# preethamam/AutomaticPanoramicImageStitching-AutoPanoStitch-MATLAB

Measured on AMD Instinct MI355X. Metric: MPix/s end-to-end stitch (SIFT->blend), 64x4K images, higher is better.
Workload: dtype f32; 1 GPU

## Files before the change

automaticpanoramicimagestitching-autopanostitch-matlab_amd/csrc/aps_internal.h:

```cpp
#pragma once
#include <hip/hip_runtime.h>
#include <type_traits>

#include <cstdarg>
#include <cstdint>
#include <cstdio>
#include <cstring>
#include <stdexcept>
#include <string>
#include <vector>

#include "../../include/aps.h"

namespace aps {

struct Error : std::exception {
    int code;
    std::string msg;
    Error(int c, std::string m) : code(c), msg(std::move(m)) {}
    const char* what() const noexcept override { return msg.c_str(); }
};

[[noreturn]] void fail(int code, const char* fmt, ...) __attribute__((format(printf, 2, 3)));
void set_last_error(const char* s);

#define APS_HIP(expr)                                                                       \
    do {                                                                                    \
        hipError_t e_ = (expr);                                                             \
        if (e_ != hipSuccess)                                                               \
            ::aps::fail(e_ == hipErrorOutOfMemory ? APS_E_OOM : APS_E_DEVICE,               \
                        "%s failed: %s (%s:%d)", #expr, hipGetErrorString(e_), __FILE__,    \
                        __LINE__);                                                          \
    } while (0)

#define APS_REQUIRE(cond, code, ...)                   \
    do {                                               \
        if (!(cond)) ::aps::fail((code), __VA_ARGS__); \
    } while (0)

template <class F>
inline int guarded(F&& f) {
    try {
        f();
        return APS_OK;
    } catch (const Error& e) {
        set_last_error(e.msg.c_str());
        return e.code;
    } catch (const std::bad_alloc&) {
        set_last_error("host allocation failed");
        return APS_E_OOM;
    } catch (const std::exception& e) {
        set_last_error(e.what());
        return APS_E_INTERNAL;
    } catch (...) {
        set_last_error("unknown exception");
        return APS_E_INTERNAL;
    }
}

struct Ctx {
    int device = -1;
    hipStream_t own_stream = nullptr;
    hipStream_t user_stream = nullptr;
    bool use_user_stream = false;
    int own_priority = 0;
    hipEvent_t ev0 = nullptr, ev1 = nullptr;
    struct Block {
        void* p;
        size_t bytes;
        bool used;
    };
    std::vector<Block> blocks;
    hipStream_t stream() const { return use_user_stream ? user_stream : own_stream; }
};

Ctx& ctx();
inline hipStream_t stream() { return ctx().stream(); }

void* ws_alloc(size_t bytes);
void ws_free(void* p);
size_t ws_idle_bytes();

template <class T>
struct Ws {
    T* p = nullptr;
    size_t n = 0;
    Ws() = default;
    explicit Ws(size_t count) { alloc(count); }
    Ws(const Ws&) = delete;
    Ws& operator=(const Ws&) = delete;
    Ws(Ws&& o) noexcept : p(o.p), n(o.n) { o.p = nullptr; }
    Ws& operator=(Ws&& o) noexcept {
        if (this != &o) {
            reset();
            p = o.p;
            n = o.n;
            o.p = nullptr;
        }
        return *this;
    }
    ~Ws() { reset(); }
    void alloc(size_t count) {
        reset();
        n = count;
        p = static_cast<T*>(ws_alloc((count ? count : 1) * sizeof(T)));
    }
    void reset() {
        if (p) ws_free(p);
        p = nullptr;
    }
    T* get() const { return p; }
    operator T*() const { return p; }
};

bool is_device_ptr(const void* p);

template <class T>
struct In {
    const T* d = nullptr;
    Ws<T> tmp;
    In() = default;
    In(const T* p, size_t count) { bind(p, count); }
    void bind(const T* p, size_t count) {
        if (count == 0 || p == nullptr) {
            d = p;
            return;
        }
        if (is_device_ptr(p)) {
            d = p;
        } else {
            tmp.alloc(count);
            APS_HIP(hipMemcpyAsync(tmp.p, p, count * sizeof(T), hipMemcpyHostToDevice, stream()));
            d = tmp.p;
        }
    }
    const T* get() const { return d; }
    operator const T*() const { return d; }
};

template <class T>
struct Out {
    T* d = nullptr;
    T* host = nullptr;
    size_t n = 0;
    Ws<T> tmp;
    Out() = default;
    Out(T* p, size_t count) { bind(p, count); }
    void bind(T* p, size_t count) {
        n = count;
        if (p == nullptr) return;
        if (count == 0 || is_device_ptr(p)) {
            d = p;
        } else {
            host = p;
            tmp.alloc(count);
            d = tmp.p;
        }
    }
    void commit(size_t count = SIZE_MAX) {
        if (!host) return;
        if (count > n) count = n;
        if (count) {
            APS_HIP(hipMemcpyAsync(host, d, count * sizeof(T), hipMemcpyDeviceToHost, stream()));
            APS_HIP(hipStreamSynchronize(stream()));
        }
    }
    void commit_2d(size_t width, size_t rows, size_t ld) {
        if (!host || width == 0 || rows == 0) return;
        if (ld == width || rows == 1) return commit(width * rows);
        APS_HIP(hipMemcpy2DAsync(host, ld * sizeof(T), d, ld * sizeof(T), width * sizeof(T), rows, hipMemcpyDeviceToHost, stream()));
        APS_HIP(hipStreamSynchronize(stream()));
    }
    T* get() const { return d; }
    operator T*() const { return d; }
    bool present() const { return d != nullptr; }
};

struct Prof {
    int slot = -1;
    void* ev_b = nullptr;
    explicit Prof(const char* name);
    ~Prof();
};

inline void check_launch(const char* what) {
    hipError_t e = hipGetLastError();
    if (e != hipSuccess) fail(APS_E_DEVICE, "launch of %s failed: %s", what, hipGetErrorString(e));
}

inline size_t matrix_extent(int64_t n, int64_t ld, int64_t cols, int layout) {
    return layout == APS_ROWMAJOR ? (size_t)(n - 1) * ld + cols : (size_t)(cols - 1) * ld + n;
}

template <class Off, class Key>
__device__ __forceinline__ int last_at_or_below_by(Off&& off, int n, Key key) {
    int lo = 0, hi = n - 1;
    while (lo < hi) {
        const int mid = (lo + hi + 1) >> 1;
        if (off(mid) <= key) lo = mid; else hi = mid - 1;
    }
    return lo;
}
template <class T, class Key>
__device__ __forceinline__ int last_at_or_below(const T* __restrict__ off, int n, Key key) {
    return last_at_or_below_by([off](int j) { return off[j]; }, n, key);
}

struct SlotTable {
    std::vector<int64_t> job_off;
    int64_t slots = 0;
};
SlotTable slot_table(const std::vector<int64_t>& off, int a, int b, bool every_j);
void screened_block_top3(const float* X_dev, int64_t ld, int layout, const std::vector<int64_t>& block_off, const SlotTable& table,
                         uint32_t* t3_idx, float* t3_d, float* t3_b);
struct GlobalSets {
    struct Impl;
    Impl* impl = nullptr;
    GlobalSets() = default;
    GlobalSets(const GlobalSets&) = delete;
    GlobalSets& operator=(const GlobalSets&) = delete;
    ~GlobalSets();
};
int64_t screened_global_top3(const float* X_dev, int64_t ld, int layout, const std::vector<int64_t>& img_off, int img_a, int img_b,
                             float ratio, const SlotTable& table, const int64_t* d_img_off, const int64_t* d_job_off, GlobalSets& sets,
                             uint32_t* t3_idx, float* t3_d, float* t3_b, uint8_t* dismissed);

struct PopcOp {
    __host__ __device__ unsigned int operator()(unsigned long long v) const {
#if defined(__HIP_DEVICE_COMPILE__)
        return (unsigned int)__popcll(v);
#else
        return (unsigned int)__builtin_popcountll(v);
#endif
    }
};

inline unsigned cdiv(size_t a, size_t b) { return static_cast<unsigned>((a + b - 1) / b); }

template <int I, int N, class F>
__device__ __forceinline__ void static_for(F&& f) {
    if constexpr (I < N) {
        f(std::integral_constant<int, I>{});
        static_for<I + 1, N>(f);
    }
}


}
```

automaticpanoramicimagestitching-autopanostitch-matlab_amd/csrc/core.hip:

```cpp
#include <atomic>
#include <cstdlib>
#include <mutex>

#include <cstring>

#include "aps_internal.h"

namespace aps {

static thread_local std::string g_err;
static thread_local Ctx g_ctx;
static std::atomic<int> g_default_device{-1};

void set_last_error(const char* s) { g_err = s ? s : ""; }

void fail(int code, const char* fmt, ...) {
    char buf[1024];
    va_list ap;
    va_start(ap, fmt);
    vsnprintf(buf, sizeof buf, fmt, ap);
    va_end(ap);
    throw Error(code, buf);
}

static bool device_is_gfx950(int dev) {
    hipDeviceProp_t prop;
    if (hipGetDeviceProperties(&prop, dev) != hipSuccess) return false;
    return std::strncmp(prop.gcnArchName, "gfx950", 6) == 0;
}

static int count_devices() {
    int n = 0;
    if (hipGetDeviceCount(&n) != hipSuccess) {
        (void)hipGetLastError();
        return 0;
    }
    int ok = 0;
    for (int i = 0; i < n; ++i)
        if (device_is_gfx950(i)) ++ok;
    return ok == n ? n : 0;
}

static void bind_device(Ctx& c, int dev) {
    int n = count_devices();
    if (n <= 0)
        fail(APS_E_DEVICE,
             "no gfx950 (MI355X) device is visible; libaps_hip has no CPU fallback by design");
    if (dev < 0 || dev >= n) fail(APS_E_ARG, "device %d out of range [0,%d)", dev, n);
    APS_HIP(hipSetDevice(dev));
    if (c.device != dev) {
        for (auto& b : c.blocks) (void)hipFree(b.p);
        c.blocks.clear();
        if (c.own_stream) (void)hipStreamDestroy(c.own_stream);
        if (c.ev0) (void)hipEventDestroy(c.ev0);
        if (c.ev1) (void)hipEventDestroy(c.ev1);
        c.own_stream = nullptr;
        c.ev0 = c.ev1 = nullptr;
        c.device = dev;
    }
    if (!c.own_stream) APS_HIP(hipStreamCreateWithFlags(&c.own_stream, hipStreamNonBlocking));
    if (!c.ev0) APS_HIP(hipEventCreate(&c.ev0));
    if (!c.ev1) APS_HIP(hipEventCreate(&c.ev1));
}

Ctx& ctx() {
    Ctx& c = g_ctx;
    if (c.device < 0) {
        int dev = g_default_device.load(std::memory_order_acquire);
        if (dev < 0) {
            dev = 0;
            if (const char* e = std::getenv("APS_DEVICE")) dev = std::atoi(e);
        }
        bind_device(c, dev);
    } else {
        APS_HIP(hipSetDevice(c.device));
    }
    return c;
}

void* ws_alloc(size_t bytes) {
    Ctx& c = ctx();
    bytes = (bytes + 255) & ~size_t(255);
    int best = -1;
    for (int i = 0; i < (int)c.blocks.size(); ++i) {
        auto& b = c.blocks[i];
        if (!b.used && b.bytes >= bytes && (best < 0 || b.bytes < c.blocks[best].bytes)) best = i;
    }
    if (best >= 0 && c.blocks[best].bytes <= 2 * bytes + (1u << 20)) {
        c.blocks[best].used = true;
        return c.blocks[best].p;
    }
    void* p = nullptr;
    hipError_t e = hipMalloc(&p, bytes);
    if (e != hipSuccess) {
        (void)hipGetLastError();
        for (auto it = c.blocks.begin(); it != c.blocks.end();) {
            if (!it->used) {
                (void)hipFree(it->p);
                it = c.blocks.erase(it);
            } else {
                ++it;
            }
        }
        e = hipMalloc(&p, bytes);
        if (e != hipSuccess) {
            (void)hipGetLastError();
            fail(APS_E_OOM, "device allocation of %zu bytes failed: %s", bytes,
                 hipGetErrorString(e));
        }
    }
    c.blocks.push_back({p, bytes, true});
    return p;
}

size_t ws_idle_bytes() {
    size_t n = 0;
    for (const auto& b : ctx().blocks)
        if (!b.used) n += b.bytes;
    return n;
}

void ws_free(void* p) {
    for (auto& b : g_ctx.blocks)
        if (b.p == p) {
            b.used = false;
            return;
        }
}

struct ProfRec {
    const char* name;
    hipEvent_t a, b;
};
static std::atomic<int> g_prof_on{0};
static std::mutex g_prof_mu;
static std::vector<ProfRec> g_prof;
static std::vector<hipEvent_t> g_prof_pool;

static hipEvent_t prof_event_locked() {
    if (!g_prof_pool.empty()) {
        hipEvent_t e = g_prof_pool.back();
        g_prof_pool.pop_back();
        return e;
    }
    hipEvent_t e;
    APS_HIP(hipEventCreate(&e));
    return e;
}

Prof::Prof(const char* name) {
    const int mode = g_prof_on.load(std::memory_order_relaxed);
    if (!mode) return;
    if (mode == 2) {
        static const char* const keep[] = {"match", "ransac", "cover", "render_", "ba_", "crop", "gain", "knn", "global_"};
        bool ok = false;
        for (const char* k : keep) ok = ok || std::strncmp(name, k, std::strlen(k)) == 0;
        if (!ok) return;
    }
    hipStream_t st = stream();
    std::lock_guard<std::mutex> lk(g_prof_mu);
    ProfRec r{name, prof_event_locked(), prof_event_locked()};
    APS_HIP(hipEventRecord(r.a, st));
    g_prof.push_back(r);
    ev_b = r.b;
    slot = 1;
}
Prof::~Prof() {
    if (slot >= 0) (void)hipEventRecord(static_cast<hipEvent_t>(ev_b), stream());
}

bool is_device_ptr(const void* p) {
    if (!p) return false;
    hipPointerAttribute_t attr;
    hipError_t e = hipPointerGetAttributes(&attr, p);
    if (e != hipSuccess) {
        (void)hipGetLastError();
        return false;
    }
    return attr.type == hipMemoryTypeDevice || attr.type == hipMemoryTypeManaged;
}

}

using namespace aps;

extern "C" {

int aps_version(void) { return APS_VERSION; }

const char* aps_last_error(void) { return g_err.c_str(); }

int aps_device_count(void) { return count_devices(); }

int aps_set_device(int device) {
    return guarded([&] {
        bind_device(g_ctx, device);
        g_default_device.store(device, std::memory_order_release);
    });
}

int aps_set_thread_device(int device) {
    return guarded([&] { bind_device(g_ctx, device); });
}

int aps_set_thread_stream_priority(int level) {
    return guarded([&] {
        Ctx& c = ctx();
        int least = 0, greatest = 0;
        APS_HIP(hipDeviceGetStreamPriorityRange(&least, &greatest));
        const int prio = level > 0 ? greatest : (level < 0 ? least : (least + greatest) / 2);
        hipStream_t fresh = nullptr;
        APS_HIP(hipStreamCreateWithPriority(&fresh, hipStreamNonBlocking, prio));
        if (c.own_stream) {
            (void)hipStreamSynchronize(c.own_stream);
            (void)hipStreamDestroy(c.own_stream);
        }
        c.own_stream = fresh;
        c.own_priority = level > 0 ? 1 : 0;
    });
}

int aps_get_device(void) {
    int dev = -1;
    const int rc = guarded([&] { dev = ctx().device; });
    return rc == APS_OK ? dev : -1;
}

int aps_set_stream(void* hip_stream) {
    return guarded([&] {
        Ctx& c = ctx();
        c.user_stream = static_cast<hipStream_t>(hip_stream);
        c.use_user_stream = true;
        if (hip_stream == nullptr) c.use_user_stream = false;
    });
}

int aps_synchronize(void) {
    return guarded([&] { APS_HIP(hipStreamSynchronize(stream())); });
}

int aps_release_workspace(void) {
    return guarded([&] {
        Ctx& c = ctx();
        APS_HIP(hipStreamSynchronize(c.stream()));
        for (auto it = c.blocks.begin(); it != c.blocks.end();) {
            if (!it->used) {
                (void)hipFree(it->p);
                it = c.blocks.erase(it);
            } else {
                ++it;
            }
        }
    });
}

int aps_profile_enable(int on) {
    return guarded([&] {
        ctx();
        g_prof_on.store(on == 2 ? 2 : (on != 0 ? 1 : 0));
    });
}

int aps_profile_reset(void) {
    return guarded([&] {
        ctx();
        APS_HIP(hipDeviceSynchronize());
        std::lock_guard<std::mutex> lk(g_prof_mu);
        for (auto& r : g_prof) {
            g_prof_pool.push_back(r.a);
            g_prof_pool.push_back(r.b);
        }
        g_prof.clear();
    });
}

int aps_profile_get(const char* name, double* total_ms, int* launches) {
    return guarded([&] {
        APS_REQUIRE(name && total_ms && launches, APS_E_ARG, "NULL argument");
        ctx();
        APS_HIP(hipDeviceSynchronize());
        std::lock_guard<std::mutex> lk(g_prof_mu);
        double t = 0;
        int n = 0;
        for (auto& r : g_prof)
            if (std::strcmp(r.name, name) == 0) {
                float ms = 0;
                APS_HIP(hipEventElapsedTime(&ms, r.a, r.b));
                t += ms;
                ++n;
            }
        *total_ms = t;
        *launches = n;
    });
}

int aps_profile_series(const char* name, double* ms, int cap, int* count) {
    return guarded([&] {
        APS_REQUIRE(name && count && cap >= 0 && (cap == 0 || ms), APS_E_ARG, "bad argument");
        ctx();
        APS_HIP(hipDeviceSynchronize());
        std::lock_guard<std::mutex> lk(g_prof_mu);
        int n = 0;
        for (auto& r : g_prof)
            if (std::strcmp(r.name, name) == 0) {
                if (n < cap) {
                    float t = 0;
                    APS_HIP(hipEventElapsedTime(&t, r.a, r.b));
                    ms[n] = t;
                }
                ++n;
            }
        *count = n;
    });
}

int aps_profile_names(char* buf, int buf_len) {
    return guarded([&] {
        APS_REQUIRE(buf && buf_len > 0, APS_E_ARG, "bad buffer");
        std::string out;
        std::vector<const char*> seen;
        std::lock_guard<std::mutex> lk(g_prof_mu);
        for (auto& r : g_prof) {
            bool dup = false;
            for (auto* s : seen) dup |= std::strcmp(s, r.name) == 0;
            if (dup) continue;
            seen.push_back(r.name);
            if (!out.empty()) out += ';';
            out += r.name;
        }
        std::snprintf(buf, buf_len, "%s", out.c_str());
    });
}

int aps_timer_begin(void) {
    return guarded([&] {
        Ctx& c = ctx();
        APS_HIP(hipEventRecord(c.ev0, c.stream()));
    });
}

int aps_timer_end(float* ms) {
    return guarded([&] {
        APS_REQUIRE(ms != nullptr, APS_E_ARG, "ms is NULL");
        Ctx& c = ctx();
        APS_HIP(hipEventRecord(c.ev1, c.stream()));
        APS_HIP(hipEventSynchronize(c.ev1));
        APS_HIP(hipEventElapsedTime(ms, c.ev0, c.ev1));
    });
}

}
```

automaticpanoramicimagestitching-autopanostitch-matlab_amd/csrc/prims_dev.h:

```cpp
#pragma once
#include <hip/hip_runtime.h>

#include "aps_internal.h"

#include <rocprim/rocprim.hpp>

namespace aps {
namespace {

template <class InIt, class T>
inline void exclusive_scan(InIt in, T* out, T init, size_t n) {
    size_t bytes = 0;
    APS_HIP(rocprim::exclusive_scan(nullptr, bytes, in, out, init, n, rocprim::plus<T>(), stream()));
    Ws<char> tmp(bytes);
    APS_HIP(rocprim::exclusive_scan(tmp.get(), bytes, in, out, init, n, rocprim::plus<T>(), stream()));
}

template <class It>
inline auto popcounts(It words) {
    return rocprim::make_transform_iterator(words, PopcOp());
}

template <class Size = size_t, class KeyIn, class KeyOut, class ValIn, class ValOut>
inline void sort_pairs(KeyIn keys, KeyOut skeys, ValIn vals, ValOut svals, unsigned int n, unsigned int key_bits) {
    size_t bytes = 0;
    APS_HIP(rocprim::radix_sort_pairs(nullptr, bytes, keys, skeys, vals, svals, (Size)n, 0u, key_bits, stream()));
    Ws<char> tmp(bytes);
    APS_HIP(rocprim::radix_sort_pairs(tmp.get(), bytes, keys, skeys, vals, svals, (Size)n, 0u, key_bits, stream()));
}

template <class T>
inline void read_back(const T* d, T* h, int k) {
    APS_HIP(hipMemcpyAsync(h, d, (size_t)k * sizeof(T), hipMemcpyDeviceToHost, stream()));
    APS_HIP(hipStreamSynchronize(stream()));
}
template <class T>
inline T read_back(const T* d) {
    T v;
    read_back(d, &v, 1);
    return v;
}

template <class T>
inline T scan_total(const T* pos, const T* val, size_t n) {
    T last_pos, last_val;
    APS_HIP(hipMemcpyAsync(&last_pos, pos + n - 1, sizeof(T), hipMemcpyDeviceToHost, stream()));
    APS_HIP(hipMemcpyAsync(&last_val, val + n - 1, sizeof(T), hipMemcpyDeviceToHost, stream()));
    APS_HIP(hipStreamSynchronize(stream()));
    return last_pos + last_val;
}

}
}
```

automaticpanoramicimagestitching-autopanostitch-matlab_amd/csrc/sift.hip:

```cpp
#include <algorithm>
#include <cmath>
#include <cstring>
#include <vector>

#include "aps_internal.h"
#include "select_dev.h"

namespace aps {

constexpr int kBorder = 5;
constexpr int kMaxInterp = 5;
constexpr int kOriBins = 36;
constexpr float kFix = 1048576.0f;

__device__ __forceinline__ long long to_fix(float v) { return (long long)(int)rintf(v * kFix); }
constexpr float kFltEps = 1.1920928955078125e-07f;

constexpr int kMaxViews = APS_SIFT_MAX_VIEWS;
constexpr int kViewShift = 44;
static_assert(kMaxViews <= 16, "the view takes 4 bits of the key");
struct ViewImgs {
    const uint8_t* p[kMaxViews];
};

__device__ __forceinline__ float poly_exp2(float f) {
    float p = 1.5252733804059841e-05f;
    p = fmaf(p, f, 1.5403530393381609e-04f);
    p = fmaf(p, f, 1.3333558146428443e-03f);
    p = fmaf(p, f, 9.6181291076284772e-03f);
    p = fmaf(p, f, 5.5504108664821580e-02f);
    p = fmaf(p, f, 2.4022650695910071e-01f);
    p = fmaf(p, f, 6.9314718055994531e-01f);
    p = fmaf(p, f, 1.0f);
    return p;
}
__device__ __forceinline__ float my_exp2(float t) {
    if (t < -125.0f) return 0.0f;
    if (t > 125.0f) t = 125.0f;
    const float n = rintf(t);
    const float p = poly_exp2(t - n);
    return p * __uint_as_float((uint32_t)((int)n + 127) << 23);
}
__device__ __forceinline__ float my_exp(float x) { return my_exp2(x * 1.4426950408889634f); }

__device__ __forceinline__ float fast_atan2_deg(float y, float x) {
    const float p1 = 0.9997878412794807f * 57.29577951308232f, p3 = -0.3258083974640975f * 57.29577951308232f;
    const float p5 = 0.1555786518463281f * 57.29577951308232f, p7 = -0.04432655554792128f * 57.29577951308232f;
    const float ax = fabsf(x), ay = fabsf(y);
    const bool steep = !(ax >= ay);
    const float c = (steep ? ax : ay) / ((steep ? ay : ax) + 2.220446049250313e-16f);
    const float c2 = c * c;
    float a = (((p7 * c2 + p5) * c2 + p3) * c2 + p1) * c;
    if (steep) a = 90.0f - a;
    if (x < 0) a = 180.0f - a;
    if (y < 0) a = 360.0f - a;
    return a;
}

__device__ __forceinline__ void sincos_deg(float a, float& s, float& c) {
    const float k = rintf(a / 90.0f);
    const float r = a - 90.0f * k;
    const float x = r * 0.017453292519943295f, x2 = x * x;
    float sp = 2.7557319223985893e-06f;
    sp = fmaf(sp, x2, -1.9841269841269841e-04f);
    sp = fmaf(sp, x2, 8.3333333333333332e-03f);
    sp = fmaf(sp, x2, -1.6666666666666666e-01f);
    sp = fmaf(sp * x2, x, x);
    float cp = -2.7557319223985888e-07f;
    cp = fmaf(cp, x2, 2.4801587301587302e-05f);
    cp = fmaf(cp, x2, -1.3888888888888889e-03f);
    cp = fmaf(cp, x2, 4.1666666666666664e-02f);
    cp = fmaf(cp, x2, -0.5f);
    cp = fmaf(cp, x2, 1.0f);
    const int q = (((int)k % 4) + 4) % 4;
    if (q == 0) {
        s = sp;
        c = cp;
    } else if (q == 1) {
        s = cp;
        c = -sp;
    } else if (q == 2) {
        s = -sp;
        c = -cp;
    } else {
        s = -cp;
        c = sp;
    }
}

__device__ __forceinline__ int reflect101(int p, int n) {
    if (n == 1) return 0;
    while (p < 0 || p >= n) {
        if (p < 0)
            p = -p;
        else
            p = 2 * (n - 1) - p;
    }
    return p;
}

constexpr int kGUW = 128, kGUH = 16;
__global__ __launch_bounds__(256) void gray_up_kernel(ViewImgs imgs, int h, int w, int c, int layout,
                                                      float* __restrict__ out_, size_t pitch) {
    const uint8_t* __restrict__ img = imgs.p[blockIdx.z];
    float* __restrict__ out = out_ + blockIdx.z * pitch;
    constexpr int GW = kGUW / 2 + 2, GH = kGUH / 2 + 2;
    __shared__ float s_g[GH][GW + 1];
    const int x0 = blockIdx.x * kGUW, y0 = blockIdx.y * kGUH;
    const int cx0 = x0 / 2 - 1, cy0 = y0 / 2 - 1;
    for (int e = threadIdx.x; e < GH * GW; e += 256) {
        const int ly = e / GW, lx = e - ly * GW;
        const int y = min(max(cy0 + ly, 0), h - 1), x = min(max(cx0 + lx, 0), w - 1);
        float v;
        if (c == 1) {
            v = (float)(layout == APS_IMG_U8_HWC ? img[(size_t)y * w + x] : img[(size_t)x * h + y]);
        } else {
            uint8_t ch[3];
#pragma unroll
            for (int k = 0; k < 3; ++k)
                ch[k] = layout == APS_IMG_U8_HWC ? img[((size_t)y * w + x) * 3 + k]
                                                 : img[(size_t)k * h * w + (size_t)x * h + y];
            const double d = 0.298936021293775 * ch[0] + 0.587043074451121 * ch[1] + 0.114020904255103 * ch[2];
            v = (float)floor(d + 0.5);
        }
        s_g[ly][lx] = v;
    }
    __syncthreads();
    const int y = y0 + threadIdx.x / 16, xb = x0 + (threadIdx.x & 15) * 8;
    if (y >= 2 * h || xb >= 2 * w) return;
    float fy = ((float)y + 0.5f) * 0.5f - 0.5f;
    int sy = (int)floorf(fy);
    fy -= (float)sy;
    if (sy < 0) {
        sy = 0;
        fy = 0;
    }
    if (sy >= h - 1) {
        sy = h - 1;
        fy = 0;
    }
    const int sy1 = sy + 1 < h ? sy + 1 : h - 1;
    const float b0 = 1.0f - fy, b1 = fy;
    const float* r0 = s_g[sy - cy0];
    const float* r1 = s_g[sy1 - cy0];
    float res[8];
#pragma unroll
    for (int j = 0; j < 8; ++j) {
        const int x = xb + j;
        float fx = ((float)x + 0.5f) * 0.5f - 0.5f;
        int sx = (int)floorf(fx);
        fx -= (float)sx;
        if (sx < 0) {
            sx = 0;
            fx = 0;
        }
        if (sx >= w - 1) {
            sx = w - 1;
            fx = 0;
        }
        const int sx1 = sx + 1 < w ? sx + 1 : w - 1;
        const float a0 = 1.0f - fx, a1 = fx;
        const float h0 = r0[sx - cx0] * a0 + r0[sx1 - cx0] * a1;
        const float h1 = r1[sx - cx0] * a0 + r1[sx1 - cx0] * a1;
        res[j] = h0 * b0 + h1 * b1;
    }
    float* dst = out + (size_t)y * (2 * w) + xb;
    if (xb + 8 <= 2 * w && (w & 1) == 0) {
        reinterpret_cast<float4*>(dst)[0] = make_float4(res[0], res[1], res[2], res[3]);
        reinterpret_cast<float4*>(dst)[1] = make_float4(res[4], res[5], res[6], res[7]);
    } else {
#pragma unroll
        for (int j = 0; j < 8; ++j)
            if (xb + j < 2 * w) dst[j] = res[j];
    }
}

__global__ void decimate_kernel(const float* __restrict__ in_, int h, int w, size_t pitch, int oh, int ow,
                                float* __restrict__ out_, size_t opitch) {
    const float* __restrict__ in = in_ + blockIdx.z * pitch;
    float* __restrict__ out = out_ + blockIdx.z * opitch;
    const int x = blockIdx.x * blockDim.x + threadIdx.x, y = blockIdx.y;
    if (x >= ow) return;
    out[(size_t)y * ow + x] = in[(size_t)min(2 * y, h - 1) * w + min(2 * x, w - 1)];
}

struct GaussK {
    float k[64];
    int n;
};

constexpr int kTW = 64, kTH = 32;

typedef float f32x2 __attribute__((ext_vector_type(2)));
template <int T>
__device__ __forceinline__ void pk_tap(f32x2& acc, const GaussK& gk, f32x2 v) {
    unsigned long long kk;
    __builtin_memcpy(&kk, &gk.k[T & ~1], sizeof kk);
    if (T & 1)
        asm("v_pk_fma_f32 %0, %1, %2, %0 op_sel:[1,0,0] op_sel_hi:[1,1,1]" : "+v"(acc) : "s"(kk), "v"(v));
    else
        asm("v_pk_fma_f32 %0, %1, %2, %0 op_sel_hi:[0,1,1]" : "+v"(acc) : "s"(kk), "v"(v));
}

template <int R>
constexpr bool kBlurOneBuffer = R >= 7;

template <int R, int TW = kTW, int NT = 256>
__device__ __forceinline__ void blur_tile_passes(const float* s_in, float* s_row, const GaussK& gk, int x0, int y0, int h, int w,
                                                 float* __restrict__ out, float* __restrict__ dec, int dh, int dw) {
    constexpr int RP = (R + 3) & ~3, OFF = RP - R;
    constexpr int IW = TW + 2 * RP, IH = kTH + 2 * R;
    constexpr int IP2 = 2 * IW + 4;
    constexpr int RPITCH = TW + 2;
    const int tid = threadIdx.x;
    __syncthreads();
    constexpr bool one_buf = kBlurOneBuffer<R>;
    static_assert(!one_buf || (IH / 2) * (TW / 8) <= NT, "one work item per thread");
    for (int u = tid; u < (one_buf ? NT : (IH / 2) * (TW / 8)); u += NT) {
        const bool live = u < (IH / 2) * (TW / 8);
        const int uc = live ? u : 0;
        const int seg = uc / (IH / 2), p = uc - seg * (IH / 2), xb = seg * 8;
        const f32x2* src = reinterpret_cast<const f32x2*>(&s_in[p * IP2 + 2 * (OFF + xb)]);
        f32x2 v[8 + 2 * R], acc[8];
#pragma unroll
        for (int j = 0; j < 8 + 2 * R; ++j) v[j] = src[j];
#pragma unroll
        for (int j = 0; j < 8; ++j) acc[j] = f32x2{0.f, 0.f};
        static_for<0, 2 * R + 1>([&](auto T) {
            constexpr int t = decltype(T)::value;
#pragma unroll
            for (int j = 0; j < 8; ++j) pk_tap<t>(acc[j], gk, v[j + t]);
        });
        if (one_buf) __syncthreads();
        float* d0 = &s_row[(2 * p) * RPITCH + xb];
        if (live) {
#pragma unroll
            for (int j = 0; j < 8; ++j) {
                d0[j] = acc[j].x;
                d0[RPITCH + j] = acc[j].y;
            }
        }
    }
    __syncthreads();
    for (int u = tid; u < (TW / 2) * (kTH / 4); u += NT) {
        const int lx = 2 * (u & (TW / 2 - 1)), yb = (u / (TW / 2)) * 4;
        f32x2 v[4 + 2 * R], acc[4];
#pragma unroll
        for (int j = 0; j < 4 + 2 * R; ++j) v[j] = *reinterpret_cast<const f32x2*>(&s_row[(yb + j) * RPITCH + lx]);
#pragma unroll
        for (int j = 0; j < 4; ++j) acc[j] = f32x2{0.f, 0.f};
        static_for<0, 2 * R + 1>([&](auto T) {
            constexpr int t = decltype(T)::value;
#pragma unroll
            for (int j = 0; j < 4; ++j) pk_tap<t>(acc[j], gk, v[j + t]);
        });
        const int gx = x0 + lx;
        if (gx + 1 < w && (w & 1) == 0) {
#pragma unroll
            for (int j = 0; j < 4; ++j) {
                const int gy = y0 + yb + j;
                if (gy < h) *reinterpret_cast<f32x2*>(&out[(size_t)gy * w + gx]) = acc[j];
            }
        } else if (gx < w) {
#pragma unroll
            for (int j = 0; j < 4; ++j) {
                const int gy = y0 + yb + j;
                if (gy < h) {
                    out[(size_t)gy * w + gx] = acc[j].x;
                    if (gx + 1 < w) out[(size_t)gy * w + gx + 1] = acc[j].y;
                }
            }
        }
        if (dec && (gx >> 1) < dw) {
#pragma unroll
            for (int j = 0; j < 4; j += 2) {
                const int dy = (y0 + yb + j) >> 1;
                if (dy < dh) dec[(size_t)dy * dw + (gx >> 1)] = acc[j].x;
            }
        }
    }
}

template <int R, int TW = kTW, int NT = 256>
__global__ __launch_bounds__(NT) void blur_kernel(const float* __restrict__ in_, int h, int w, GaussK gk,
                                                   float* __restrict__ out_, float* __restrict__ dec_, int dh, int dw,
                                                   size_t pitch, size_t dpitch) {
    const float* __restrict__ in = in_ + blockIdx.z * pitch;
    float* __restrict__ out = out_ + blockIdx.z * pitch;
    float* __restrict__ dec = dec_ ? dec_ + blockIdx.z * dpitch : nullptr;
    constexpr int RP = (R + 3) & ~3;
    constexpr int IW = TW + 2 * RP, IH = kTH + 2 * R, NV = IW / 4;
    static_assert(IH % 2 == 0 && kTH % 4 == 0, "row pairs");
    constexpr int IP2 = 2 * IW + 4;
    constexpr int RPITCH = TW + 2;
    static_assert((IP2 / 4) % 2 == 1, "pitch");
    static_assert(IH * RPITCH <= (IH / 2) * IP2, "the row-pass result fits the tile's buffer");
    __shared__ __attribute__((aligned(16))) float s_in[(IH / 2) * IP2];
    __shared__ __attribute__((aligned(16))) float s_row_own[kBlurOneBuffer<R> ? 1 : IH * RPITCH];
    float* const s_row = kBlurOneBuffer<R> ? s_in : s_row_own;
    const int x0 = blockIdx.x * TW, y0 = blockIdx.y * kTH;
    const int tid = threadIdx.x;
    const bool vec_ok = (w & 3) == 0 && (reinterpret_cast<uintptr_t>(in) & 15) == 0;
    constexpr int NPF = (IH * NV + NT - 1) / NT;
    float4 pf[NPF];
// ... 967 lines not shown
        default: return false;
    }
    check_launch("blur_base_kernel");
    return true;
}

static int num_octaves(int H, int W) {
    const int mn = std::min(2 * W, 2 * H);
    return (int)std::lrint(std::log((double)mn) / std::log(2.0) - 2.0) + 1;
}


static void check_sift_args(const aps_sift_view* views, int nv, int height, int width, int channels, int img_layout,
                            const aps_sift_params* params, int desc_layout) {
    APS_REQUIRE(views && params, APS_E_ARG, "NULL argument");
    APS_REQUIRE(nv >= 1 && nv <= kMaxViews, APS_E_ARG, "n_views must be in 1..%d", kMaxViews);
    for (int v = 0; v < nv; ++v) APS_REQUIRE(views[v].img, APS_E_ARG, "NULL argument");
    APS_REQUIRE(height > 0 && width > 0, APS_E_DIM, "empty image");
    APS_REQUIRE(channels == 1 || channels == 3, APS_E_DIM, "channels must be 1 or 3");
    APS_REQUIRE(img_layout == APS_IMG_U8_HWC || img_layout == APS_IMG_U8_MATLAB, APS_E_TYPE, "unknown image layout");
    APS_REQUIRE(desc_layout == APS_ROWMAJOR || desc_layout == APS_COLMAJOR, APS_E_TYPE, "unknown descriptor layout");
    APS_REQUIRE(params->n_layers >= 1 && params->n_layers <= 5, APS_E_ARG, "NumLayersInOctave must be in 1..5");
    APS_REQUIRE(params->sigma > 0.5, APS_E_ARG, "Sigma must exceed the assumed camera blur 0.5");
    APS_REQUIRE(params->contrast_threshold >= 0 && params->edge_threshold >= 1, APS_E_ARG, "bad thresholds");
    for (int v = 0; v < nv; ++v) APS_REQUIRE(views[v].cap >= 0, APS_E_ARG, "negative capacity");
    APS_REQUIRE(2 * (int64_t)height < 65536 && 2 * (int64_t)width < 65536, APS_E_DIM, "image side must be < 32768");
}

struct Pyramid {
    int nv = 0;
    std::vector<Ws<float>> G;
    std::vector<PyrTable> table;
    Ws<PyrTable> d_table;
};

static void build_pyramid(const ViewImgs& imgs, int nv, int H, int W, int channels, int img_layout, const aps_sift_params* params,
                          int n_oct, Pyramid& P) {
    const int nl = params->n_layers;
    Ws<float> up, scratch;
    Ws<uint8_t> gray8;
    std::vector<Ws<float>>& G = P.G;
    G = std::vector<Ws<float>>((size_t)n_oct * (nl + 3));
    P.nv = nv;
    P.table.assign(nv, PyrTable());
    std::memset(P.table.data(), 0, nv * sizeof(PyrTable));
    for (PyrTable& t : P.table) {
        t.n_oct = n_oct;
        t.nl = nl;
        t.sigma = (float)params->sigma;
    }
    double sig[16];
    sig[0] = params->sigma;
    const double kf = std::pow(2.0, 1.0 / nl);
    for (int i = 1; i < nl + 3; ++i) {
        const double sp = std::pow(kf, (double)(i - 1)) * params->sigma, st = sp * kf;
        sig[i] = std::sqrt(st * st - sp * sp);
    }
    int ow = 2 * W, oh = 2 * H, pw = 0, ph = 0;
    bool base_written = false;
    for (int o = 0; o < n_oct; ++o) {
        if (o > 0) {
            pw = ow;
            ph = oh;
            ow = std::max(1, ow / 2);
            oh = std::max(1, oh / 2);
        }
        const size_t pitch = view_pitch(ow, oh);
        for (int i = 0; i < nl + 3; ++i)
            if (!(i == 0 && base_written)) G[o * (nl + 3) + i].alloc(nv * pitch);
        if (o == 0) {
            double sd = params->sigma * params->sigma - 4.0 * 0.5 * 0.5;
            if (sd < 0.01) sd = 0.01;
            if (!launch_base_blur(nv, imgs, H, W, channels, img_layout, std::sqrt(sd), G[0], gray8)) {
                up.alloc(nv * pitch);
                gray_up_kernel<<<dim3(cdiv(2 * W, kGUW), cdiv(2 * H, kGUH), nv), 256, 0, stream()>>>(imgs, H, W, channels, img_layout, up, pitch);
                check_launch("gray_up_kernel");
                launch_blur(nv, up, oh, ow, std::sqrt(sd), G[0], scratch);
            }
        } else if (!base_written) {
            decimate_kernel<<<dim3(cdiv(ow, 256), oh, nv), 256, 0, stream()>>>(G[(o - 1) * (nl + 3) + nl], ph, pw, view_pitch(pw, ph), oh, ow,
                                                                            G[o * (nl + 3)], pitch);
            check_launch("decimate_kernel");
        }
        base_written = false;
        for (int i = 1; i < nl + 3; ++i) {
            if (i == nl && o + 1 < n_oct) {
                const int nw = std::max(1, ow / 2), nh = std::max(1, oh / 2);
                G[(o + 1) * (nl + 3)].alloc(nv * view_pitch(nw, nh));
                base_written = launch_blur(nv, G[o * (nl + 3) + i - 1], oh, ow, sig[i], G[o * (nl + 3) + i], scratch,
                                           G[(o + 1) * (nl + 3)], nh, nw);
            } else {
                launch_blur(nv, G[o * (nl + 3) + i - 1], oh, ow, sig[i], G[o * (nl + 3) + i], scratch);
            }
        }
        for (int v = 0; v < nv; ++v) {
            OctaveDesc& od = P.table[v].oct[o];
            od.w = ow;
            od.h = oh;
            for (int i = 0; i < nl + 3; ++i) od.G[i] = G[o * (nl + 3) + i].get() + v * pitch;
        }
    }
    P.d_table.alloc(nv);
    APS_HIP(hipMemcpyAsync(P.d_table, P.table.data(), nv * sizeof(PyrTable), hipMemcpyHostToDevice, stream()));
}

static unsigned int detect_candidates(const Pyramid& P, const aps_sift_params* params, int H, int W, Ws<KpRec>& recs, unsigned int* n_cand) {
    const PyrTable& table = P.table[0];
    const int nl = table.nl, n_oct = table.n_oct, nv = P.nv;
    const unsigned int cand_cap = (unsigned int)std::min<size_t>(
        params->max_features > 0 ? (size_t)params->max_features : std::max<size_t>((size_t)H * W / 2, 65536), 1u << 26);
    unsigned int cells_cap = (unsigned int)std::min<size_t>(std::max<size_t>((size_t)H * W / 2, 1u << 18), 1u << 27);
    Ws<unsigned long long> cells((size_t)nv * cells_cap);
    recs.alloc((size_t)nv * cand_cap);
    Ws<unsigned int> d_count(2 * nv);
    unsigned int h_count[2 * kMaxViews];
    const float thr = (float)(int)std::floor(0.5 * params->contrast_threshold / nl * 255.0);
    unsigned int max_cells = 0;
    for (int attempt = 0; attempt < 2; ++attempt) {
        APS_HIP(hipMemsetAsync(d_count, 0, 2 * nv * sizeof(unsigned int), stream()));
        ExtremaWavePlan plan;
        std::memset(&plan, 0, sizeof plan);
        int run = 0;
        for (int o = 0; o < 16; ++o) {
            plan.job_ptr[o] = run;
            plan.nstrip[o] = plan.ch[o] = 1;
            if (o >= n_oct) continue;
            const OctaveDesc& od = table.oct[o];
            if (od.w <= 2 * kBorder || od.h <= 2 * kBorder) continue;
            const int ns = cdiv(od.w, kWS);
            int ch = (int)(((long long)od.h * ns + 8191) / 8192);
            ch = std::max(24, ch);
            plan.nstrip[o] = ns;
            plan.ch[o] = ch;
            run += ns * cdiv(od.h, ch);
        }
        plan.job_ptr[16] = run;
        if (run > 0) {
            Prof prof("sift_extrema");
            const dim3 wgs(cdiv(run, 4), nv);
            switch (nl) {
                case 1: extrema_wave_kernel<1><<<wgs, 256, 0, stream()>>>(P.d_table, plan, thr, cells, d_count, cells_cap); break;
                case 2: extrema_wave_kernel<2><<<wgs, 256, 0, stream()>>>(P.d_table, plan, thr, cells, d_count, cells_cap); break;
                case 3: extrema_wave_kernel<3><<<wgs, 256, 0, stream()>>>(P.d_table, plan, thr, cells, d_count, cells_cap); break;
                case 4: extrema_wave_kernel<4><<<wgs, 256, 0, stream()>>>(P.d_table, plan, thr, cells, d_count, cells_cap); break;
                default: extrema_wave_kernel<5><<<wgs, 256, 0, stream()>>>(P.d_table, plan, thr, cells, d_count, cells_cap); break;
            }
            check_launch("extrema_wave_kernel");
        }
        read_back(d_count.get(), h_count, 2 * nv);
        max_cells = 0;
        for (int v = 0; v < nv; ++v) max_cells = std::max(max_cells, h_count[2 * v]);
        if (max_cells <= cells_cap) break;
        APS_REQUIRE(attempt == 0, APS_E_INTERNAL, "extrema count changed between identical sweeps");
        cells_cap = max_cells;
        cells.alloc((size_t)nv * cells_cap);
    }
    if (max_cells > 0) {
        Prof prof("sift_refine");
        refine_kernel<<<dim3(cdiv(max_cells, 256), nv), 256, 0, stream()>>>(P.d_table, cells, d_count, cells_cap,
                                                                            (float)params->contrast_threshold,
                                                                            (float)params->edge_threshold, recs, d_count.get() + 1,
                                                                            cand_cap);
        check_launch("refine_kernel");
    }
    read_back(d_count.get(), h_count, 2 * nv);
    for (int v = 0; v < nv; ++v) {
        n_cand[v] = h_count[2 * v + 1];
        if (n_cand[v] > cand_cap)
            fail(APS_E_CAP, "SIFT found %u extrema, more than the candidate capacity %u (raise params.max_features)", n_cand[v], cand_cap);
    }
    return cand_cap;
}

static unsigned int segment_counts(const unsigned int* pos, const unsigned int* val, const Segments& seg, int nv, unsigned int* count) {
    Ws<unsigned int> d_ends(nv);
    unsigned int ends[kMaxViews];
    segment_ends_kernel<<<1, 64, 0, stream()>>>(pos, val, seg, nv, d_ends);
    check_launch("segment_ends_kernel");
    read_back(d_ends.get(), ends, nv);
    for (int v = 0; v < nv; ++v) count[v] = ends[v] - (v ? ends[v - 1] : 0u);
    return ends[nv - 1];
}

static Segments segments_of(const unsigned int* count, int nv) {
    Segments seg;
    std::memset(&seg, 0, sizeof seg);
    for (int v = 0; v < kMaxViews; ++v) seg.off[v + 1] = seg.off[v] + (v < nv ? count[v] : 0u);
    return seg;
}

static unsigned int canonical_keypoints(const Ws<KpRec>& recs, unsigned int cand_cap, const unsigned int* n_cand, int nv, Ws<KpRec>& kps,
                                        unsigned int* n_kp) {
    const Segments seg = segments_of(n_cand, nv);
    const unsigned int n = seg.off[nv], most = *std::max_element(n_cand, n_cand + nv);
    Ws<unsigned long long> keys(n), keys_s(n);
    Ws<unsigned int> idx(n), idx_s(n), flag(n), pos(n);
    rec_keys_kernel<<<dim3(cdiv(most, 256), nv), 256, 0, stream()>>>(recs, cand_cap, seg, keys, idx);
    sort_pairs<unsigned int>(keys.get(), keys_s.get(), idx.get(), idx_s.get(), n, nv > 1 ? kViewShift + 4u : (unsigned int)kViewShift);
    unique_flag_kernel<<<cdiv(n, 256), 256, 0, stream()>>>(keys_s, n, flag);
    exclusive_scan(flag.get(), pos.get(), 0u, n);
    const unsigned int total = segment_counts(pos, flag, seg, nv, n_kp);
    kps.alloc(total);
    compact_recs_kernel<<<cdiv(n, 256), 256, 0, stream()>>>(recs, idx_s, flag, pos, n, kps);
    check_launch("compact_recs_kernel");
    return total;
}

struct Orientations {
    Ws<unsigned int> ocount, opos;
    Ws<float> oangle;
};

static unsigned int orient_keypoints(const Pyramid& P, const Ws<KpRec>& kps, const unsigned int* n_kp, unsigned int n, Orientations& O,
                                     unsigned int* n_rows) {
    O.ocount.alloc(n);
    O.opos.alloc(n);
    O.oangle.alloc((size_t)n * kOriBins);
    Ws<unsigned char> obin((size_t)n * kOriBins);
    {
        Prof prof("sift_orient");
        orient_kernel<<<cdiv(n, 4), 256, 0, stream()>>>(P.d_table, kps, n, O.ocount, O.oangle, obin);
    }
    check_launch("orient_kernel");
    exclusive_scan(O.ocount.get(), O.opos.get(), 0u, n);
    return segment_counts(O.opos, O.ocount, segments_of(n_kp, P.nv), P.nv, n_rows);
}

static Ws<OrientedKp> select_rows(const Ws<KpRec>& kps, unsigned int n_kp, const Orientations& O, unsigned int n_all, unsigned int n_out,
                                  const unsigned int* n_view_out, int nv, int H, int W, int grid_rows, int grid_cols) {
    Ws<OrientedKp> oks_all(n_all);
    expand_oriented_kernel<<<cdiv(n_kp, 256), 256, 0, stream()>>>(O.ocount, O.opos, O.oangle, n_kp, oks_all);
    check_launch("expand_oriented_kernel");
    if (n_out == n_all) return oks_all;
    Prof prof("sift_select");
    Ws<unsigned long long> skeys(n_all), words;
    Ws<unsigned int> svals(n_all), sprefix;
    unsigned int n_words = 0;
    if (grid_rows > 0 || nv > 1) {
        const int rows = grid_rows > 0 ? grid_rows : 1, cols = grid_rows > 0 ? grid_cols : 1;
        sift_uniform_key_kernel<<<cdiv(n_all, 256), 256, 0, stream()>>>(kps, oks_all, n_all, H, W, rows, cols, skeys, svals);
        check_launch("sift_uniform_key_kernel");
        UniformBudget budget = {};
        for (int v = 0; v < nv; ++v) budget.q[v] = n_view_out[v];
        select_uniform(skeys, nullptr, svals, n_all, (unsigned int)nv, (unsigned int)(rows * cols), budget, words, sprefix, n_words);
    } else {
        sift_contr_key_kernel<<<cdiv(n_all, 256), 256, 0, stream()>>>(kps, oks_all, n_all, skeys, svals);
        check_launch("sift_contr_key_kernel");
        select_by_key(skeys, svals, n_all, single_group_cut(n_all, n_out), words, sprefix, n_words, 32u);
    }
    Ws<OrientedKp> oks_sel(n_out);
    select_compact_kernel<OrientedKp><<<cdiv(n_words, 256), 256, 0, stream()>>>(words, sprefix, n_words, oks_all, n_all, oks_sel, n_out);
    check_launch("select_compact_kernel");
    return oks_sel;
}

static void describe(const Pyramid& P, const Ws<KpRec>& kps, const Ws<OrientedKp>& oks, const unsigned int* n_out, unsigned int n,
                     aps_sift_view* views, int desc_layout, int64_t ldd, int64_t ldl) {
    const int nv = P.nv;
    for (int v = 0; v < nv; ++v) {
        if (n_out[v] == 0) continue;
        APS_REQUIRE(views[v].desc && views[v].loc, APS_E_ARG, "NULL output with features present");
        if (desc_layout == APS_ROWMAJOR)
            APS_REQUIRE(ldd >= 128, APS_E_DIM, "ldd < 128");
        else
            APS_REQUIRE(ldd >= n_out[v], APS_E_DIM, "ldd < count");
        APS_REQUIRE(ldl >= n_out[v], APS_E_DIM, "ldl < count");
    }
    std::vector<Out<float>> odesc(nv), oaux(nv);
    std::vector<Out<double>> oloc(nv);
    ViewDst dst[kMaxViews];
    std::memset(dst, 0, sizeof dst);
    unsigned int row0 = 0;
    for (int v = 0; v < nv; ++v) {
        dst[v].row0 = row0;
        row0 += n_out[v];
        if (n_out[v] == 0) continue;
        const size_t desc_elems = desc_layout == APS_ROWMAJOR ? (size_t)(n_out[v] - 1) * ldd + 128 : (size_t)127 * ldd + n_out[v];
        odesc[v].bind(views[v].desc, desc_elems);
        oaux[v].bind(views[v].aux, (size_t)n_out[v] * 4);
        oloc[v].bind(views[v].loc, (size_t)ldl + n_out[v]);
        dst[v].desc = odesc[v];
        dst[v].loc = oloc[v];
        dst[v].aux = oaux[v].present() ? oaux[v].get() : nullptr;
    }
    Ws<ViewDst> d_dst(nv);
    APS_HIP(hipMemcpyAsync(d_dst, dst, nv * sizeof(ViewDst), hipMemcpyHostToDevice, stream()));
    {
        Prof prof("sift_descr");
        descr_kernel<<<cdiv(n, 4), 256, 0, stream()>>>(P.d_table, kps, oks, n, d_dst, desc_layout, ldd, ldl);
    }
    check_launch("descr_kernel");
    for (int v = 0; v < nv; ++v) {
        if (n_out[v] == 0) continue;
        if (desc_layout == APS_ROWMAJOR)
            odesc[v].commit_2d(128, n_out[v], (size_t)ldd);
        else
            odesc[v].commit_2d(n_out[v], 128, (size_t)ldd);
        oloc[v].commit_2d(n_out[v], 2, (size_t)ldl);
        oaux[v].commit();
    }
    APS_HIP(hipStreamSynchronize(stream()));
}

}

using namespace aps;

static void sift_chain(aps_sift_view* views, int nv, int height, int width, int channels, int img_layout, const aps_sift_params* params,
                       long long n_strongest, int grid_rows, int grid_cols, int desc_layout, int64_t ldd, int64_t ldl) {
    check_sift_args(views, nv, height, width, channels, img_layout, params, desc_layout);
    ctx();
    for (int v = 0; v < nv; ++v) views[v].count = 0;
    const int H = height, W = width;
    std::vector<In<uint8_t>> dimg(nv);
    ViewImgs imgs;
    std::memset(&imgs, 0, sizeof imgs);
    for (int v = 0; v < nv; ++v) {
        dimg[v].bind(views[v].img, (size_t)H * W * channels);
        imgs.p[v] = dimg[v];
    }
    const int n_oct = std::min(num_octaves(H, W), 16);
    if (n_oct <= 0) return;
    Pyramid pyr;
    build_pyramid(imgs, nv, H, W, channels, img_layout, params, n_oct, pyr);
    Ws<KpRec> recs, kps;
    unsigned int n_cand[kMaxViews], n_kp[kMaxViews], n_all[kMaxViews], n_out[kMaxViews];
    const unsigned int cand_cap = detect_candidates(pyr, params, H, W, recs, n_cand);
    if (*std::max_element(n_cand, n_cand + nv) == 0) return;
    const unsigned int n_kp_sum = canonical_keypoints(recs, cand_cap, n_cand, nv, kps, n_kp);
    Orientations ori;
    const unsigned int n_all_sum = orient_keypoints(pyr, kps, n_kp, n_kp_sum, ori, n_all);
    unsigned int n_out_sum = 0;
    bool fits = true;
    for (int v = 0; v < nv; ++v) {
        n_out[v] = n_strongest > 0 ? (unsigned int)std::min<long long>(n_all[v], n_strongest) : n_all[v];
        n_out_sum += n_out[v];
        views[v].count = n_out[v];
        fits = fits && (int64_t)n_out[v] <= views[v].cap;
    }
    for (int v = 0; v < nv && !fits; ++v)
        if ((int64_t)n_out[v] > views[v].cap) fail(APS_E_CAP, "feature capacity %lld < %u features", (long long)views[v].cap, n_out[v]);
    if (n_out_sum == 0) return;
    const Ws<OrientedKp> oks = select_rows(kps, n_kp_sum, ori, n_all_sum, n_out_sum, n_out, nv, H, W, grid_rows, grid_cols);
    describe(pyr, kps, oks, n_out, n_out_sum, views, desc_layout, ldd, ldl);
}

static void sift_single(const uint8_t* img, int height, int width, int channels, int img_layout, const aps_sift_params* params,
                        long long n_strongest, int grid_rows, int grid_cols, float* desc, int desc_layout, int64_t ldd, double* loc,
                        int64_t ldl, float* aux, int64_t cap, int64_t* count) {
    APS_REQUIRE(img && params && count, APS_E_ARG, "NULL argument");
    aps_sift_view view = {img, desc, loc, aux, cap, *count};
    try {
        sift_chain(&view, 1, height, width, channels, img_layout, params, n_strongest, grid_rows, grid_cols, desc_layout, ldd, ldl);
    } catch (...) {
        *count = view.count;
        throw;
    }
    *count = view.count;
}

extern "C" {

int aps_sift_extract(const uint8_t* img, int height, int width, int channels, int img_layout,
                     const aps_sift_params* params, float* desc, int desc_layout, int64_t ldd,
                     double* loc, int64_t ldl, float* aux, int64_t cap, int64_t* count) {
    return guarded([&] { sift_single(img, height, width, channels, img_layout, params, 0, 0, 0, desc, desc_layout, ldd, loc, ldl, aux, cap, count); });
}

int aps_sift_extract_batch(aps_sift_view* views, int n_views, int height, int width, int channels, int img_layout,
                           const aps_sift_params* params, int desc_layout, int64_t ldd, int64_t ldl) {
    return guarded([&] { sift_chain(views, n_views, height, width, channels, img_layout, params, 0, 0, 0, desc_layout, ldd, ldl); });
}

int aps_sift_extract_batch_strongest(aps_sift_view* views, int n_views, int height, int width, int channels, int img_layout,
                                     const aps_sift_strongest_params* params, int desc_layout, int64_t ldd, int64_t ldl) {
    return guarded([&] {
        APS_REQUIRE(params, APS_E_ARG, "NULL argument");
        APS_REQUIRE(params->n_strongest >= 1, APS_E_ARG, "n_strongest (NumStrongest) must be at least 1");
        sift_chain(views, n_views, height, width, channels, img_layout, &params->sift, params->n_strongest, 0, 0, desc_layout, ldd, ldl);
    });
}

int aps_sift_extract_batch_uniform(aps_sift_view* views, int n_views, int height, int width, int channels, int img_layout,
                                   const aps_sift_uniform_params* params, int desc_layout, int64_t ldd, int64_t ldl) {
    return guarded([&] {
        APS_REQUIRE(params, APS_E_ARG, "NULL argument");
        check_uniform(params->strongest.n_strongest, params->grid_rows, params->grid_cols);
        sift_chain(views, n_views, height, width, channels, img_layout, &params->strongest.sift, params->strongest.n_strongest,
                   params->grid_rows, params->grid_cols, desc_layout, ldd, ldl);
    });
}

int aps_sift_extract_strongest(const uint8_t* img, int height, int width, int channels, int img_layout,
                               const aps_sift_strongest_params* params, float* desc, int desc_layout, int64_t ldd,
                               double* loc, int64_t ldl, float* aux, int64_t cap, int64_t* count) {
    return guarded([&] {
        APS_REQUIRE(params, APS_E_ARG, "NULL argument");
        APS_REQUIRE(params->n_strongest >= 1, APS_E_ARG, "n_strongest (NumStrongest) must be at least 1");
        sift_single(img, height, width, channels, img_layout, &params->sift, params->n_strongest, 0, 0, desc, desc_layout, ldd, loc, ldl, aux,
                    cap, count);
    });
}

int aps_sift_extract_uniform(const uint8_t* img, int height, int width, int channels, int img_layout,
                             const aps_sift_uniform_params* params, float* desc, int desc_layout, int64_t ldd,
                             double* loc, int64_t ldl, float* aux, int64_t cap, int64_t* count) {
    return guarded([&] {
        APS_REQUIRE(params, APS_E_ARG, "NULL argument");
        check_uniform(params->strongest.n_strongest, params->grid_rows, params->grid_cols);
        sift_single(img, height, width, channels, img_layout, &params->strongest.sift, params->strongest.n_strongest, params->grid_rows,
                    params->grid_cols, desc, desc_layout, ldd, loc, ldl, aux, cap, count);
    });
}

}
```

Measured before the change: 3480 MPix/s.

## Pipeline SIFT pyramid builds against keypoint chains on two streams

Batches of more than eight views are split into chunks. The Gaussian pyramid for the next chunk is built on the main stream while the current chunk's detection, orientation and descriptor chain runs on a new side stream, with events ordering the two. Host read-backs inside the chain go through a pinned buffer and an event wait, so they do not stall the main stream. The workspace allocator tags blocks by stream to avoid cross-stream reuse hazards. Smaller per-launch batches and the extra synchronisation may offset the overlap.

```diff
diff --git a/automaticpanoramicimagestitching-autopanostitch-matlab_amd/csrc/aps_internal.h b/automaticpanoramicimagestitching-autopanostitch-matlab_amd/csrc/aps_internal.h
--- a/automaticpanoramicimagestitching-autopanostitch-matlab_amd/csrc/aps_internal.h
+++ b/automaticpanoramicimagestitching-autopanostitch-matlab_amd/csrc/aps_internal.h
@@ -69,13 +69,35 @@
         void* p;
         size_t bytes;
         bool used;
+        hipStream_t last;
     };
     std::vector<Block> blocks;
-    hipStream_t stream() const { return use_user_stream ? user_stream : own_stream; }
+    hipStream_t side_stream = nullptr;
+    hipEvent_t ev_ready[2] = {nullptr, nullptr}, ev_read = nullptr;
+    void* pinned = nullptr;
+    bool two_streams = false;
+    hipStream_t cur = nullptr;
+    hipStream_t main_stream() const { return use_user_stream ? user_stream : own_stream; }
+    hipStream_t stream() const { return two_streams ? cur : main_stream(); }
 };
 
 Ctx& ctx();
 inline hipStream_t stream() { return ctx().stream(); }
+
+struct TwoStreams {
+    TwoStreams();
+    ~TwoStreams();
+    TwoStreams(const TwoStreams&) = delete;
+    TwoStreams& operator=(const TwoStreams&) = delete;
+    void on_main();
+    void on_side();
+    void publish(int i);
+    void await(int i);
+    void drain_side();
+    void finish();
+};
+constexpr size_t kReadBackBytes = 4096;
+void two_stream_read_back(const void* d, void* h, size_t bytes);
 
 void* ws_alloc(size_t bytes);
 void ws_free(void* p);
diff --git a/automaticpanoramicimagestitching-autopanostitch-matlab_amd/csrc/core.hip b/automaticpanoramicimagestitching-autopanostitch-matlab_amd/csrc/core.hip
--- a/automaticpanoramicimagestitching-autopanostitch-matlab_amd/csrc/core.hip
+++ b/automaticpanoramicimagestitching-autopanostitch-matlab_amd/csrc/core.hip
@@ -13,6 +13,19 @@
 static std::atomic<int> g_default_device{-1};
 
 void set_last_error(const char* s) { g_err = s ? s : ""; }
+
+static void drain_two_streams(Ctx& c) {
+    (void)hipStreamSynchronize(c.main_stream());
+    if (c.side_stream) (void)hipStreamSynchronize(c.side_stream);
+}
+
+static void drop_side_stream(Ctx& c) {
+    if (c.side_stream) {
+        (void)hipStreamSynchronize(c.side_stream);
+        (void)hipStreamDestroy(c.side_stream);
+    }
+    c.side_stream = nullptr;
+}
 
 void fail(int code, const char* fmt, ...) {
     char buf[1024];
@@ -20,6 +33,7 @@
     va_start(ap, fmt);
     vsnprintf(buf, sizeof buf, fmt, ap);
     va_end(ap);
+    if (g_ctx.two_streams) drain_two_streams(g_ctx);
     throw Error(code, buf);
 }
 
@@ -54,6 +68,13 @@
         if (c.own_stream) (void)hipStreamDestroy(c.own_stream);
         if (c.ev0) (void)hipEventDestroy(c.ev0);
         if (c.ev1) (void)hipEventDestroy(c.ev1);
+        drop_side_stream(c);
+        for (hipEvent_t* e : {&c.ev_ready[0], &c.ev_ready[1], &c.ev_read}) {
+            if (*e) (void)hipEventDestroy(*e);
+            *e = nullptr;
+        }
+        if (c.pinned) (void)hipHostFree(c.pinned);
+        c.pinned = nullptr;
         c.own_stream = nullptr;
         c.ev0 = c.ev1 = nullptr;
         c.device = dev;
@@ -84,10 +105,12 @@
     int best = -1;
     for (int i = 0; i < (int)c.blocks.size(); ++i) {
         auto& b = c.blocks[i];
+        if (c.two_streams && b.last && b.last != c.cur) continue;
         if (!b.used && b.bytes >= bytes && (best < 0 || b.bytes < c.blocks[best].bytes)) best = i;
     }
     if (best >= 0 && c.blocks[best].bytes <= 2 * bytes + (1u << 20)) {
         c.blocks[best].used = true;
+        if (c.two_streams) c.blocks[best].last = c.cur;
         return c.blocks[best].p;
     }
     void* p = nullptr;
@@ -109,7 +132,7 @@
                  hipGetErrorString(e));
         }
     }
-    c.blocks.push_back({p, bytes, true});
+    c.blocks.push_back({p, bytes, true, c.two_streams ? c.cur : nullptr});
     return p;
 }
 
@@ -167,6 +190,46 @@
 }
 Prof::~Prof() {
     if (slot >= 0) (void)hipEventRecord(static_cast<hipEvent_t>(ev_b), stream());
+}
+
+TwoStreams::TwoStreams() {
+    Ctx& c = ctx();
+    APS_REQUIRE(!c.two_streams, APS_E_INTERNAL, "nested two-stream call");
+    if (!c.side_stream) {
+        int prio = 0;
+        APS_HIP(hipStreamGetPriority(c.main_stream(), &prio));
+        APS_HIP(hipStreamCreateWithPriority(&c.side_stream, hipStreamNonBlocking, prio));
+    }
+    for (hipEvent_t* e : {&c.ev_ready[0], &c.ev_ready[1], &c.ev_read})
+        if (!*e) APS_HIP(hipEventCreateWithFlags(e, hipEventDisableTiming));
+    if (!c.pinned) APS_HIP(hipHostMalloc(&c.pinned, kReadBackBytes, hipHostMallocDefault));
+    c.cur = c.main_stream();
+    c.two_streams = true;
+}
+TwoStreams::~TwoStreams() {
+    Ctx& c = g_ctx;
+    drain_two_streams(c);
+    for (auto& b : c.blocks) b.last = nullptr;
+    c.two_streams = false;
+    c.cur = nullptr;
+}
+void TwoStreams::on_main() { g_ctx.cur = g_ctx.main_stream(); }
+void TwoStreams::on_side() { g_ctx.cur = g_ctx.side_stream; }
+void TwoStreams::publish(int i) { APS_HIP(hipEventRecord(g_ctx.ev_ready[i], g_ctx.main_stream())); }
+void TwoStreams::await(int i) { APS_HIP(hipStreamWaitEvent(g_ctx.side_stream, g_ctx.ev_ready[i], 0)); }
+void TwoStreams::drain_side() { APS_HIP(hipStreamSynchronize(g_ctx.side_stream)); }
+void TwoStreams::finish() {
+    APS_HIP(hipStreamSynchronize(g_ctx.main_stream()));
+    APS_HIP(hipStreamSynchronize(g_ctx.side_stream));
+}
+
+void two_stream_read_back(const void* d, void* h, size_t bytes) {
+    Ctx& c = ctx();
+    APS_REQUIRE(c.two_streams && bytes <= kReadBackBytes, APS_E_INTERNAL, "read-back of %zu bytes outside its room", bytes);
+    APS_HIP(hipMemcpyAsync(c.pinned, d, bytes, hipMemcpyDeviceToHost, c.cur));
+    APS_HIP(hipEventRecord(c.ev_read, c.cur));
+    APS_HIP(hipEventSynchronize(c.ev_read));
+    std::memcpy(h, c.pinned, bytes);
 }
 
 bool is_device_ptr(const void* p) {
@@ -217,6 +280,7 @@
         }
         c.own_stream = fresh;
         c.own_priority = level > 0 ? 1 : 0;
+        drop_side_stream(c);
     });
 }
 
diff --git a/automaticpanoramicimagestitching-autopanostitch-matlab_amd/csrc/prims_dev.h b/automaticpanoramicimagestitching-autopanostitch-matlab_amd/csrc/prims_dev.h
--- a/automaticpanoramicimagestitching-autopanostitch-matlab_amd/csrc/prims_dev.h
+++ b/automaticpanoramicimagestitching-autopanostitch-matlab_amd/csrc/prims_dev.h
@@ -31,6 +31,7 @@
 
 template <class T>
 inline void read_back(const T* d, T* h, int k) {
+    if (ctx().two_streams) return two_stream_read_back(d, h, (size_t)k * sizeof(T));
     APS_HIP(hipMemcpyAsync(h, d, (size_t)k * sizeof(T), hipMemcpyDeviceToHost, stream()));
     APS_HIP(hipStreamSynchronize(stream()));
 }
diff --git a/automaticpanoramicimagestitching-autopanostitch-matlab_amd/csrc/sift.hip b/automaticpanoramicimagestitching-autopanostitch-matlab_amd/csrc/sift.hip
--- a/automaticpanoramicimagestitching-autopanostitch-matlab_amd/csrc/sift.hip
+++ b/automaticpanoramicimagestitching-autopanostitch-matlab_amd/csrc/sift.hip
@@ -1,5 +1,6 @@
 #include <algorithm>
 #include <cmath>
+#include <cstdlib>
 #include <cstring>
 #include <vector>
 
@@ -1573,6 +1574,46 @@
     APS_HIP(hipStreamSynchronize(stream()));
 }
 
+static bool keypoint_chain(const Pyramid& pyr, aps_sift_view* views, int H, int W, const aps_sift_params* params, long long n_strongest,
+                           int grid_rows, int grid_cols, int desc_layout, int64_t ldd, int64_t ldl, bool write) {
+    const int nv = pyr.nv;
+    Ws<KpRec> recs, kps;
+    unsigned int n_cand[kMaxViews], n_kp[kMaxViews], n_all[kMaxViews], n_out[kMaxViews];
+    const unsigned int cand_cap = detect_candidates(pyr, params, H, W, recs, n_cand);
+    if (*std::max_element(n_cand, n_cand + nv) == 0) return true;
+    const unsigned int n_kp_sum = canonical_keypoints(recs, cand_cap, n_cand, nv, kps, n_kp);
+    Orientations ori;
+    const unsigned int n_all_sum = orient_keypoints(pyr, kps, n_kp, n_kp_sum, ori, n_all);
+    unsigned int n_out_sum = 0;
+    bool fits = true;
+    for (int v = 0; v < nv; ++v) {
+        n_out[v] = n_strongest > 0 ? (unsigned int)std::min<long long>(n_all[v], n_strongest) : n_all[v];
+        n_out_sum += n_out[v];
+        views[v].count = n_out[v];
+        fits = fits && (int64_t)n_out[v] <= views[v].cap;
+    }
+    if (!fits) return false;
+    if (n_out_sum == 0 || !write) return true;
+    const Ws<OrientedKp> oks = select_rows(kps, n_kp_sum, ori, n_all_sum, n_out_sum, n_out, nv, H, W, grid_rows, grid_cols);
+    describe(pyr, kps, oks, n_out, n_out_sum, views, desc_layout, ldd, ldl);
+    return true;
+}
+
+static void fail_over_capacity(const aps_sift_view* views, int nv) {
+    for (int v = 0; v < nv; ++v)
+        if (views[v].count > views[v].cap)
+            fail(APS_E_CAP, "feature capacity %lld < %u features", (long long)views[v].cap, (unsigned int)views[v].count);
+}
+
+static int sift_half_views() {
+    static const int half = [] {
+        const char* e = std::getenv("APS_SIFT_HALF");
+        const int h = e ? std::atoi(e) : 8;
+        return std::min(std::max(h, 1), kMaxViews);
+    }();
+    return half;
+}
+
 }
 
 using namespace aps;
@@ -1592,28 +1633,41 @@
     }
     const int n_oct = std::min(num_octaves(H, W), 16);
     if (n_oct <= 0) return;
-    Pyramid pyr;
-    build_pyramid(imgs, nv, H, W, channels, img_layout, params, n_oct, pyr);
-    Ws<KpRec> recs, kps;
-    unsigned int n_cand[kMaxViews], n_kp[kMaxViews], n_all[kMaxViews], n_out[kMaxViews];
-    const unsigned int cand_cap = detect_candidates(pyr, params, H, W, recs, n_cand);
-    if (*std::max_element(n_cand, n_cand + nv) == 0) return;
-    const unsigned int n_kp_sum = canonical_keypoints(recs, cand_cap, n_cand, nv, kps, n_kp);
-    Orientations ori;
-    const unsigned int n_all_sum = orient_keypoints(pyr, kps, n_kp, n_kp_sum, ori, n_all);
-    unsigned int n_out_sum = 0;
+    const int half = sift_half_views();
+    if (nv <= half) {
+        Pyramid pyr;
+        build_pyramid(imgs, nv, H, W, channels, img_layout, params, n_oct, pyr);
+        if (!keypoint_chain(pyr, views, H, W, params, n_strongest, grid_rows, grid_cols, desc_layout, ldd, ldl, true))
+            fail_over_capacity(views, nv);
+        return;
+    }
+    const int n_half = (nv + half - 1) / half;
     bool fits = true;
-    for (int v = 0; v < nv; ++v) {
-        n_out[v] = n_strongest > 0 ? (unsigned int)std::min<long long>(n_all[v], n_strongest) : n_all[v];
-        n_out_sum += n_out[v];
-        views[v].count = n_out[v];
-        fits = fits && (int64_t)n_out[v] <= views[v].cap;
-    }
-    for (int v = 0; v < nv && !fits; ++v)
-        if ((int64_t)n_out[v] > views[v].cap) fail(APS_E_CAP, "feature capacity %lld < %u features", (long long)views[v].cap, n_out[v]);
-    if (n_out_sum == 0) return;
-    const Ws<OrientedKp> oks = select_rows(kps, n_kp_sum, ori, n_all_sum, n_out_sum, n_out, nv, H, W, grid_rows, grid_cols);
-    describe(pyr, kps, oks, n_out, n_out_sum, views, desc_layout, ldd, ldl);
+    {
+        TwoStreams streams;
+        Pyramid pyr[2];
+        const auto build = [&](int k) {
+            const int first = k * half, n = std::min(half, nv - first);
+            ViewImgs part;
+            std::memset(&part, 0, sizeof part);
+            for (int v = 0; v < n; ++v) part.p[v] = imgs.p[first + v];
+            streams.on_main();
+            build_pyramid(part, n, H, W, channels, img_layout, params, n_oct, pyr[k & 1]);
+            streams.publish(k & 1);
+        };
+        build(0);
+        for (int k = 0; k < n_half; ++k) {
+            if (k + 1 < n_half) build(k + 1);
+            streams.on_side();
+            streams.await(k & 1);
+            fits = keypoint_chain(pyr[k & 1], views + k * half, H, W, params, n_strongest, grid_rows, grid_cols, desc_layout, ldd, ldl,
+                                  fits) && fits;
+            streams.drain_side();
+            pyr[k & 1] = Pyramid();
+        }
+        streams.finish();
+    }
+    if (!fits) fail_over_capacity(views, nv);
 }
 
 static void sift_single(const uint8_t* img, int height, int width, int channels, int img_layout, const aps_sift_params* params,
```

Measured after the change: 3435 MPix/s. 1.3% lower.
